# guptakhil/show-tell

Hardware: AMD Instinct MI355X
Metric: training images/sec (ResNet101+GRU, emb=512, bs=128) at 1/2/4/8 MI355X (higher is better)
Workload: dtype bf16; 1 GPU; BASELINE configs[1]: ResNet-101 (train-mode BN, frozen) + 5-layer GRU decoder, E=H=512, V=10000, fwd+bwd+SGD step, synthetic COCO-shaped batch; batch_per_gpu=128, global_batch=128, image=3x224x224, parallelism=dp1

## Files before the change

### show-tell_amd/csrc/rnn.cpp

```cpp
#include "common.h"
#include "rnn_kernels.h"
#include <string.h>
#include <vector>

namespace {

inline size_t al(size_t v) { return (v + 255) & ~(size_t)255; }
inline int up8(int v) { return (v + 7) & ~7; }

struct Plan {
  int G, GH, Np, Vp, maxw;
  size_t es;
  size_t x0, y, gates, cst, dyl, dx0, dgx, dgh, dhc, dcc, tA, tB, wT, wThh, wTih, gA, gB, total;
};

Plan make_plan(const st_rnn_params* p, const st_packed_seq* s) {
  Plan q;
  q.G = p->cell == ST_CELL_GRU ? 3 : 4;
  q.GH = q.G * p->H;
  q.Np = up8(s->ntok);
  q.Vp = st_rnn_vocab_ld(p->V);
  q.es = st_dtype_size(p->dtype);
  q.maxw = p->in0 > p->H ? p->in0 : p->H;
  const size_t n = s->ntok, L = p->L, H = p->H;
  size_t o = 0;
  auto take = [&](size_t bytes) { size_t r = o; o += al(bytes); return r; };
  q.x0 = take(n * p->in0 * q.es);
  q.y = take(L * n * H * q.es);
  q.gates = take(L * n * 4 * H * q.es);
  q.cst = take(p->cell == ST_CELL_LSTM ? L * n * H * q.es : 0);
  q.dyl = take(L * n * H * sizeof(float));
  q.dx0 = take(n * p->in0 * sizeof(float));
  q.dgx = take(L * n * q.GH * q.es);
  q.dgh = take(p->cell == ST_CELL_GRU ? L * n * q.GH * q.es : 0);
  q.dhc = take(L * (size_t)s->B * H * sizeof(float));
  q.dcc = take(L * (size_t)s->B * H * sizeof(float));
  const size_t ra = (size_t)(p->V > q.GH ? p->V : q.GH);
  q.tA = take(ra * q.Np * q.es);
  q.tB = take((size_t)q.maxw * q.Np * q.es);
  const size_t w1 = (size_t)H * q.Vp, w2 = (size_t)q.maxw * q.GH;
  q.wT = take((w1 > w2 ? w1 : w2) * q.es);
  q.wThh = take(L * H * q.GH * q.es);
  q.wTih = take(L * (size_t)q.maxw * q.GH * q.es);
  q.gA = take(2 * L * (size_t)q.GH * q.Np * q.es);
  q.gB = take(2 * L * (size_t)q.maxw * q.Np * q.es);
  q.total = o;
  return q;
}

int gemm_nt(const void* a, int lda, const void* w, int ldw, void* y, int ldy, int M, int N, int K, int dtype, int out_dtype,
            const float* bias, int accumulate, void* stream, int split_k = 0) {
  if (M <= 0 || N <= 0) return 0;
  st_conv_desc d;
  memset(&d, 0, sizeof(d));
  d.split_k = split_k;
  d.x = a; d.w = w; d.y = y; d.bias = bias; d.dtype = dtype; d.out_dtype = out_dtype;
  d.B = M; d.Hin = 1; d.Win = 1; d.Cin = K; d.Ho = 1; d.Wo = 1; d.N = N; d.KH = 1; d.KW = 1; d.stride = 1; d.pad = 0;
  d.ldx = lda; d.ldw = ldw; d.ldy = ldy; d.accumulate = accumulate;
  return st_conv(&d, stream);
}

int check_common(const st_rnn_params* p, const st_packed_seq* s, const char* who) {
  ST_CHECK(p && s, "%s: null descriptor", who);
  ST_CHECK(p->cell == ST_CELL_GRU || p->cell == ST_CELL_LSTM, "%s: bad cell %d", who, p->cell);
  ST_CHECK(p->dtype == ST_F32 || p->dtype == ST_BF16, "%s: bad dtype %d", who, p->dtype);
  ST_CHECK(p->L >= 1 && p->L <= ST_MAX_LAYERS, "%s: num_layers=%d out of range [1,%d]", who, p->L, ST_MAX_LAYERS);
  ST_CHECK(p->H % 8 == 0 && p->in0 % 8 == 0 && p->E % 8 == 0, "%s: E=%d, in0=%d and H=%d must be multiples of 8", who, p->E, p->in0, p->H);
  ST_CHECK(p->V > 0, "%s: bad vocabulary size", who);
  ST_CHECK(s->B > 0 && s->T > 0 && s->ntok > 0 && s->batch_sizes_host && s->rows_b && s->rows_t && s->prev_row && s->caption,
           "%s: bad packed-sequence descriptor", who);
  int sum = 0, prev = s->B;
  for (int t = 0; t < s->T; ++t) {
    const int b = s->batch_sizes_host[t];
    ST_CHECK(b > 0 && b <= prev, "%s: batch_sizes must be positive and non-increasing (captions sorted by length, utils.py:66)", who);
    prev = b; sum += b;
  }
  ST_CHECK(sum == s->ntok && s->batch_sizes_host[0] == s->B, "%s: batch_sizes do not add up to ntok", who);
  for (int l = 0; l < p->L; ++l)
    ST_CHECK(p->w_ih[l] && p->w_hh[l] && p->b_ih[l] && p->b_hh[l], "%s: null weights for layer %d", who, l);
  return 0;
}

}

// ... 75 lines not shown
  ST_CHECK(workspace && targets && scratch && loss_accum, "st_rnn_fused_loss: null pointer");
  ST_CHECK(st_rnn_fused_loss_supported(p), "st_rnn_fused_loss: needs bf16, H = 512 and the vocabulary projection (use st_rnn_forward's logits + st_cross_entropy)");
  const Plan q = make_plan(p, s);
  ST_CHECK(workspace_bytes >= q.total && scratch_bytes >= st_rnn_fused_loss_bytes(p, s), "st_rnn_fused_loss: workspace / scratch too small");
  const char* ytop = reinterpret_cast<const char*>(workspace) + q.y + (size_t)(p->L - 1) * s->ntok * p->H * q.es;
  const int n = s->ntok;
  return vocab_ce_forward(ytop, p->w_lin, p->b_lin, targets, n, p->V, scratch + 2 * (size_t)n, scratch + n, scratch, loss_accum,
                          reinterpret_cast<hipStream_t>(stream));
}
extern "C" int st_rnn_fused_dlogits(const st_rnn_params* p, const st_packed_seq* s, const void* workspace, size_t workspace_bytes,
                                    const long* targets, const float* scratch, const float* grad_scale_dev, void* dlogits, int ldd, void* stream) {
  if (check_common(p, s, "st_rnn_fused_dlogits")) return 1;
  ST_CHECK(workspace && targets && scratch && dlogits, "st_rnn_fused_dlogits: null pointer");
  ST_CHECK(st_rnn_fused_loss_supported(p), "st_rnn_fused_dlogits: unsupported configuration");
  const Plan q = make_plan(p, s);
  ST_CHECK(workspace_bytes >= q.total, "st_rnn_fused_dlogits: workspace too small");
  const char* ytop = reinterpret_cast<const char*>(workspace) + q.y + (size_t)(p->L - 1) * s->ntok * p->H * q.es;
  return vocab_ce_dlogits(ytop, p->w_lin, p->b_lin, targets, scratch, s->ntok, p->V, dlogits, ldd, 1.0f, grad_scale_dev,
                          reinterpret_cast<hipStream_t>(stream));
}

extern "C" int st_rnn_backward(const st_rnn_params* p, const st_rnn_grads* g, const st_packed_seq* s,
                               const void* x0_override, const void* dlogits, int ldd, const float* dy_top_extra,
                               void* workspace, size_t workspace_bytes, float* dfeat, float* dx0_out, void* stream) {
  if (check_common(p, s, "st_rnn_backward")) return 1;
  ST_CHECK(g && workspace, "st_rnn_backward: null pointer");
  const Plan q = make_plan(p, s);
  ST_CHECK(workspace_bytes >= q.total, "st_rnn_backward: workspace too small (%zu < %zu)", workspace_bytes, q.total);
  hipStream_t st = reinterpret_cast<hipStream_t>(stream);
  char* ws = reinterpret_cast<char*>(workspace);
  const int dt = p->dtype, H = p->H, n = s->ntok, Np = q.Np, GH = q.GH;
  const size_t es = q.es;
  std::vector<int> off(s->T + 1, 0);
  for (int t = 0; t < s->T; ++t) off[t + 1] = off[t] + s->batch_sizes_host[t];
  const int L = p->L, T = s->T;
  auto dyl = [&](int l) { return reinterpret_cast<float*>(ws + q.dyl) + (size_t)l * n * H; };
  float* dy = dyl(L - 1);
  const char* ytop = ws + q.y + (size_t)(p->L - 1) * n * H * es;

  if (dlogits) {
    ST_CHECK(p->w_lin && g->w_lin && g->b_lin, "st_rnn_backward: vocabulary projection gradients requested without buffers");
    ST_CHECK(ldd >= up8(p->V) && ldd % 8 == 0 && ldd <= q.Vp, "st_rnn_backward: dlogits leading dimension %d must be a multiple of 8 in [%d, %d]",
             ldd, up8(p->V), q.Vp);
    if (st_transpose_colsum(dlogits, ws + q.tA, g->b_lin, dt, n, p->V, ldd, Np, stream)) return 1;
    if (st_transpose(ytop, ws + q.tB, dt, n, H, H, Np, stream)) return 1;
    if (gemm_nt(ws + q.tA, Np, ws + q.tB, Np, g->w_lin, H, p->V, H, Np, dt, ST_F32, nullptr, 1, stream)) return 1;
    if (st_transpose(p->w_lin, ws + q.wT, dt, p->V, H, H, ldd, stream)) return 1;
    const int bk = dt == ST_BF16 ? 64 : 32;
    const int split = (ldd % (8 * bk) == 0 && ldd >= 16 * bk) ? 8 : 0;
    if (gemm_nt(dlogits, ldd, ws + q.wT, ldd, dy, H, n, H, ldd, dt, ST_F32, nullptr, 0, stream, split)) return 1;
    if (dy_top_extra) { st_set_error("st_rnn_backward: dlogits and dy_top_extra are exclusive"); return 1; }
  } else {
    ST_CHECK(dy_top_extra, "st_rnn_backward: need dlogits or dy_top");
    if (hipMemcpyAsync(dy, dy_top_extra, (size_t)n * H * sizeof(float), hipMemcpyDeviceToDevice, st) != hipSuccess) {
      st_set_error("st_rnn_backward: copy failed"); return 1;
    }
  }

  const void* x0 = x0_override ? x0_override : ws + q.x0;
  const bool need_dx0 = dfeat || dx0_out || g->emb;
  float* dx0 = dx0_out ? dx0_out : reinterpret_cast<float*>(ws + q.dx0);
  const bool gru = p->cell == ST_CELL_GRU;
  auto dgxl = [&](int l) { return ws + q.dgx + (size_t)l * n * GH * es; };
  auto dghl = [&](int l) { return gru ? ws + q.dgh + (size_t)l * n * GH * es : dgxl(l); };
  auto dhcl = [&](int l) { return reinterpret_cast<float*>(ws + q.dhc) + (size_t)l * s->B * H; };
  auto dccl = [&](int l) { return reinterpret_cast<float*>(ws + q.dcc) + (size_t)l * s->B * H; };
  auto wThh = [&](int l) { return ws + q.wThh + (size_t)l * H * GH * es; };
  auto wTih = [&](int l) { return ws + q.wTih + (size_t)l * q.maxw * GH * es; };
  if (hipMemsetAsync(ws + q.dhc, 0, (size_t)L * s->B * H * sizeof(float), st) != hipSuccess ||
      hipMemsetAsync(ws + q.dcc, 0, (size_t)L * s->B * H * sizeof(float), st) != hipSuccess) { st_set_error("memset failed"); return 1; }
  {
    const void* wx[2][ST_MAX_LAYERS]; void* wy[2][ST_MAX_LAYERS];
    int ni = 0;
    for (int l = 0; l < L; ++l) {
      const int in = l == 0 ? p->in0 : H;
      wx[0][l] = p->w_hh[l]; wy[0][l] = wThh(l);
      if (!(l > 0 || need_dx0)) continue;
      if (in == H) { wx[1][ni] = p->w_ih[l]; wy[1][ni] = wTih(l); ++ni; }
      else if (st_transpose(p->w_ih[l], wTih(l), dt, GH, in, in, GH, stream)) return 1;
    }
    if (st_transpose_batch(wx[0], wy[0], nullptr, L, dt, GH, H, H, GH, nullptr, nullptr, stream)) return 1;
    if (ni && st_transpose_batch(wx[1], wy[1], nullptr, ni, dt, GH, H, H, GH, nullptr, nullptr, stream)) return 1;
  }
  for (int d = T + L - 2; d >= 0; --d) {
    RnnBwdCell gc[ST_MAX_LAYERS];
    RnnGemmArgs mc[2 * ST_MAX_LAYERS];
    int ng = 0, nm = 0;
    for (int l = d < T ? 0 : d - (T - 1); l <= d && l < L; ++l) {
      const int t = d - l;
      const int bt = s->batch_sizes_host[t];
      const int in = l == 0 ? p->in0 : H;
      char* yl = ws + q.y + (size_t)l * n * H * es;
      char* gl = ws + q.gates + (size_t)l * n * 4 * H * es;
      char* cl = ws + q.cst + (size_t)l * n * H * es;
      RnnBwdCell& c = gc[ng++];
      memset(&c, 0, sizeof(c));
      c.dy = dyl(l) + (size_t)off[t] * H; c.dhc = dhcl(l); c.dcc = dccl(l);
      c.cache = gl + (size_t)off[t] * 4 * H * es;
      c.hprev = t > 0 ? yl + (size_t)off[t - 1] * H * es : nullptr;
      c.cnew = cl + (size_t)off[t] * H * es;
      c.cprev = t > 0 ? cl + (size_t)off[t - 1] * H * es : nullptr;
      c.dgx = dgxl(l) + (size_t)off[t] * GH * es; c.dgh = dghl(l) + (size_t)off[t] * GH * es; c.Bt = bt;
      if (t > 0) {
        RnnGemmArgs& a = mc[nm++];
        memset(&a, 0, sizeof(a));
        a.A = dghl(l) + (size_t)off[t] * GH * es; a.W = wThh(l); a.M = bt; a.N = H; a.K = GH; a.lda = GH; a.ldw = GH;
        a.out_f32 = dhcl(l); a.ldo = H; a.accumulate = 1;
      }
      if (l > 0 || need_dx0) {
        RnnGemmArgs& a = mc[nm++];
        memset(&a, 0, sizeof(a));
        a.A = dgxl(l) + (size_t)off[t] * GH * es; a.W = wTih(l); a.M = bt; a.N = in; a.K = GH; a.lda = GH; a.ldw = GH;
        a.out_f32 = (l > 0 ? dyl(l - 1) + (size_t)off[t] * H : dx0 + (size_t)off[t] * in); a.ldo = in;
      }
    }
    if (rnn_bwd_gates_launch_batch(gc, ng, H, p->cell, dt, st)) return 1;
    if (rnn_gemm_launch_batch(mc, nm, dt, 0, 0, st)) return 1;
  }
  st_conv_desc gd[2 * ST_MAX_LAYERS];
  int ng = 0;
  auto wgrad = [&](const void* aT, const void* bT, float* dw, int rows, int cols) {
    st_conv_desc& d = gd[ng++];
    memset(&d, 0, sizeof(d));
    d.x = aT; d.w = bT; d.y = dw; d.dtype = dt; d.out_dtype = ST_F32;
    d.B = rows; d.Hin = 1; d.Win = 1; d.Cin = Np; d.Ho = 1; d.Wo = 1; d.N = cols; d.KH = 1; d.KW = 1; d.stride = 1; d.pad = 0;
    d.ldx = Np; d.ldw = Np; d.ldy = cols; d.accumulate = 1;
  };
  const void* tx[4][ST_MAX_LAYERS]; void* ty[4][ST_MAX_LAYERS]; float* tc[4][ST_MAX_LAYERS];
  int nx = 0;
  for (int l = 0; l < L; ++l) {
    const int in = l == 0 ? p->in0 : H;
    const char* xl = l == 0 ? reinterpret_cast<const char*>(x0) : ws + q.y + (size_t)(l - 1) * n * H * es;
    char* aIh = ws + q.gA + (size_t)(2 * l) * GH * Np * es;
    char* aHh = ws + q.gA + (size_t)(2 * l + 1) * GH * Np * es;
    char* bIh = ws + q.gB + (size_t)(2 * l) * q.maxw * Np * es;
    char* bHh = ws + q.gB + (size_t)(2 * l + 1) * q.maxw * Np * es;
    tx[0][l] = dgxl(l); ty[0][l] = aIh; tc[0][l] = g->b_ih[l];
    tx[2][l] = dghl(l); ty[2][l] = aHh; tc[2][l] = g->b_hh[l];
    tx[3][l] = ws + q.y + (size_t)l * n * H * es; ty[3][l] = bHh; tc[3][l] = nullptr;
    if (in == H) {
      tx[1][nx] = xl; ty[1][nx] = bIh; tc[1][nx] = nullptr; ++nx;
      wgrad(aIh, bIh, g->w_ih[l], GH, in);
    } else {
      if (st_transpose(xl, bIh, dt, n, in, in, Np, stream)) return 1;
    }
    wgrad(gru ? aHh : aIh, bHh, g->w_hh[l], GH, H);
    if (!gru && colsum_launch(dghl(l), g->b_hh[l], n, GH, GH, dt, st)) return 1;
  }
  if (st_transpose_batch(tx[0], ty[0], tc[0], L, dt, n, GH, GH, Np, nullptr, nullptr, stream)) return 1;
  if (nx && st_transpose_batch(tx[1], ty[1], nullptr, nx, dt, n, H, H, Np, nullptr, nullptr, stream)) return 1;
  if (gru && st_transpose_batch(tx[2], ty[2], tc[2], L, dt, n, GH, GH, Np, nullptr, nullptr, stream)) return 1;
  if (st_transpose_batch(tx[3], ty[3], nullptr, L, dt, n, H, H, Np, s->rows_t, s->prev_row, stream)) return 1;
  for (int l = 0; l < L; ++l) {
    const int in = l == 0 ? p->in0 : H;
    if (in != H && gemm_nt(ws + q.gA + (size_t)(2 * l) * GH * Np * es, Np, ws + q.gB + (size_t)(2 * l) * q.maxw * Np * es, Np,
                           g->w_ih[l], in, GH, in, Np, dt, ST_F32, nullptr, 1, stream)) return 1;
  }
  for (int i = 0; i < ng; i += 12) {
    if (st_conv_batch(gd + i, ng - i < 12 ? ng - i : 12, stream)) return 1;
  }
  if (need_dx0 && !x0_override) {
    ST_CHECK(g->emb, "st_rnn_backward: embedding gradient buffer missing");
    if (embedding_bwd_launch(dx0, s->caption, s->Tcap, s->rows_b, s->rows_t, dfeat, g->emb, n, p->E, p->V, 0, st)) return 1;
  }
  return 0;
}
```

### show-tell_amd/csrc/rnn_kernels.h

```cpp
#pragma once
#include "common.h"

struct RnnGemmArgs {
  const void* A; const void* W; int M, N, K, lda, ldw, gstride;
  const void* A2; const void* W2; int K2, lda2, ldw2;
  float* out_f32; int ldo; int accumulate;
  const float* bias_h; const float* bias_x;
  const void* gx; int ldgx;
  const void* hprev; const void* cprev; int ldhp;
  void* hout; void* cout; int ldho;
  void* hout2; int ldho2;
  void* cache; int ldcache;
  unsigned long long* argmax_keys;
  const unsigned long long* x_keys; int x_V;
  long* ids_out; int ids_stride, ids_t;
};
constexpr int kCellRawOut = 1, kCellSplit = 2;

constexpr int kRnnBatch = 16;
struct RnnGemmBatch { RnnGemmArgs c[kRnnBatch]; };
static_assert(sizeof(RnnGemmBatch) <= 4000, "kernel-argument segment is 4 KiB");
struct RnnBwdCell {
  const float* dy; float* dhc; float* dcc; const void* cache; const void* hprev; const void* cnew; const void* cprev;
  void* dgx; void* dgh; int Bt;
};
struct RnnBwdBatch { RnnBwdCell c[kRnnBatch]; };

#ifdef __HIPCC__
__device__ __forceinline__ float st_sigm(float x) { return 1.0f / (1.0f + expf(-x)); }
__device__ __forceinline__ float st_gru_unit(float xr, float xz, float xn, float hr, float hz, float hn, float hprev, float& r, float& z, float& n) {
  r = st_sigm(xr + hr);
  z = st_sigm(xz + hz);
  n = tanhf(__builtin_fmaf(r, hn, xn));
  return __builtin_fmaf(z, hprev, (1.f - z) * n);
}
__device__ __forceinline__ float st_lstm_unit(float pi, float pf, float pg, float po, float cprev, float& ig, float& fg, float& gg, float& og, float& cn) {
  ig = st_sigm(pi); fg = st_sigm(pf); gg = tanhf(pg); og = st_sigm(po);
  cn = __builtin_fmaf(fg, cprev, ig * gg);
  return og * tanhf(cn);
}
#endif

size_t rnn_greedy_pipe_bytes(const st_rnn_params* p, int B, int steps);
int rnn_greedy_pipe(const st_rnn_params* p, const void* feat, int B, int steps, void* ws, size_t ws_bytes, long* ids_out, hipStream_t st);

int vocab_ce_supported(int dtype, int H);
int vocab_ce_tiles(int V);
int vocab_ce_forward(const void* y, const void* w, const float* bias, const long* target, int n, int V, float* partial, float* tgt,
                     float* lse, float* loss, hipStream_t st);
int vocab_ce_dlogits(const void* y, const void* w, const float* bias, const long* target, const float* lse, int n, int V,
                     void* dlogits, int ldd, float gscale, const float* gscale_dev, hipStream_t st);

int rnn_gemm_launch(const RnnGemmArgs& a, int dtype, int epi, int has_x, hipStream_t st);
int rnn_gemm_launch_batch(const RnnGemmArgs* cells, int ncells, int dtype, int epi, int has_x, hipStream_t st);
int rnn_bwd_gates_launch_batch(const RnnBwdCell* cells, int ncells, int H, int cell_kind, int dtype, hipStream_t st);
int pack_inputs_launch(const void* feat, const void* emb, const long* cap, int Tcap, const int* rows_b, const int* rows_t,
                       void* x0, long* target, int ntok, int E, int V, int mode, int dtype, hipStream_t st);
int embedding_bwd_launch(const float* dx0, const long* cap, int Tcap, const int* rows_b, const int* rows_t,
                         float* dfeat, float* demb, int ntok, int E, int V, int mode, hipStream_t st);
int gather_hprev_launch(const void* y, const int* rows_t, const int* prev_row, void* hp, int ntok, int H, int dtype, hipStream_t st,
                        const void* h0 = nullptr, const int* rows_b = nullptr);
int gru_bwd_gates_launch(const float* dy, float* dhc, const void* cache, const void* hprev, void* dgx, void* dgh,
                         int Bt, int H, int dtype, hipStream_t st);
int lstm_bwd_gates_launch(const float* dy, float* dhc, float* dcc, const void* cache, const void* cnew, const void* cprev,
                          void* dg, int Bt, int H, int dtype, hipStream_t st);
int colsum_launch(const void* x, float* out, int rows, int cols, int ldx, int dtype, hipStream_t st);
```

### show-tell_amd/csrc/rnn_kernels.hip

```cpp
#include "common.h"
#include "rnn_kernels.h"
#include <string.h>

namespace {

template <typename T> struct Mfma;
template <> struct Mfma<bf16_t> {
  static constexpr int EPC = 8;
  static __device__ __forceinline__ void run(const u32x4& a, const u32x4& b, f32x4& c) {
    c = __builtin_amdgcn_mfma_f32_16x16x32_bf16(*reinterpret_cast<const bf16x8*>(&a),
                                                *reinterpret_cast<const bf16x8*>(&b), c, 0, 0, 0);
  }
};
template <> struct Mfma<float> {
  static constexpr int EPC = 4;
  static __device__ __forceinline__ void run(const u32x4& a, const u32x4& b, f32x4& c) {
#pragma unroll
    for (int e = 0; e < 4; ++e)
      c = __builtin_amdgcn_mfma_f32_16x16x4f32(__uint_as_float(a[e]), __uint_as_float(b[e]), c, 0, 0, 0);
  }
};

template <typename T> __device__ __forceinline__ void load4(const T* p, float* v);
template <> __device__ __forceinline__ void load4<float>(const float* p, float* v) {
  const f32x4 t = *reinterpret_cast<const f32x4*>(p);
  v[0] = t[0]; v[1] = t[1]; v[2] = t[2]; v[3] = t[3];
}
template <> __device__ __forceinline__ void load4<bf16_t>(const bf16_t* p, float* v) {
  const u32x2 t = *reinterpret_cast<const u32x2*>(p);
  v[0] = __uint_as_float(t[0] << 16); v[1] = __uint_as_float(t[0] & 0xffff0000u);
  v[2] = __uint_as_float(t[1] << 16); v[3] = __uint_as_float(t[1] & 0xffff0000u);
}
template <typename T> __device__ __forceinline__ void store4(T* p, const float* v);
template <> __device__ __forceinline__ void store4<float>(float* p, const float* v) {
  *reinterpret_cast<f32x4*>(p) = f32x4{v[0], v[1], v[2], v[3]};
}
template <> __device__ __forceinline__ void store4<bf16_t>(bf16_t* p, const float* v) {
  *reinterpret_cast<u32x2*>(p) = u32x2{pack_bf16x2(v[0], v[1]), pack_bf16x2(v[2], v[3])};
}

__device__ __forceinline__ float sigm(float x) { return 1.0f / (1.0f + expf(-x)); }

template <typename T, int NG, bool HAS_X, int MT>
__device__ __forceinline__ void skinny_mma(const RnnGemmArgs& a, int mbase, int n0, int r16, int q4, int kslice,
                                           f32x4 (&accH)[MT][NG], f32x4 (&accX)[MT][NG]) {
  constexpr int EPC = Mfma<T>::EPC;
  constexpr int UNR = (HAS_X && MT == 2) ? 2 : 4;
  const int n = n0 + r16;
  const bool nok = n < a.N;
  const bool hasH = a.A != nullptr, hasX = HAS_X && a.A2 != nullptr;
  const T* WH = reinterpret_cast<const T*>(a.W) + (long)n * a.ldw;
  const long gsH = (long)a.gstride * a.ldw;
  const T* WX = reinterpret_cast<const T*>(a.W2) + (long)n * a.ldw2;
  const long gsX = (long)a.gstride * a.ldw2;
  const T* AH[MT]; const T* AX[MT]; bool mok[MT];
#pragma unroll
  for (int t = 0; t < MT; ++t) {
    const int m = mbase + t * 16 + r16;
    mok[t] = m < a.M;
    AH[t] = reinterpret_cast<const T*>(a.A) + (long)m * a.lda;
    if (!HAS_X && a.x_keys && a.A) {
      int tok = 0;
      if (mok[t]) {
        tok = (int)(0xffffffffu - (unsigned)(a.x_keys[m] & 0xffffffffull));
        if (tok < 0 || tok >= a.x_V) tok = 0;
        if (a.ids_out && n0 == 0 && kslice == 0 && q4 == 0) a.ids_out[(long)m * a.ids_stride + a.ids_t] = tok;
      }
      AH[t] = reinterpret_cast<const T*>(a.A) + (long)tok * a.lda;
    }
    long xrow = m;
    if (HAS_X && a.x_keys) {
      int tok = 0;
      if (mok[t]) {
        tok = (int)(0xffffffffu - (unsigned)(a.x_keys[m] & 0xffffffffull));
        if (tok < 0 || tok >= a.x_V) tok = 0;
        if (a.ids_out && n0 == 0 && kslice == 0 && q4 == 0) a.ids_out[(long)m * a.ids_stride + a.ids_t] = tok;
      }
      xrow = tok;
    }
    AX[t] = reinterpret_cast<const T*>(a.A2) + xrow * a.lda2;
  }
  const int nsH = hasH ? (a.K + 4 * EPC - 1) / (4 * EPC) : 0, nsX = hasX ? (a.K2 + 4 * EPC - 1) / (4 * EPC) : 0;
  const int spwH = (nsH + 3) / 4, spwX = (nsX + 3) / 4;
  const int begH = kslice * spwH, endH = min(nsH, begH + spwH), begX = kslice * spwX, endX = min(nsX, begX + spwX);
  const int ngroups = max((endH - begH + UNR - 1) / UNR, (endX - begX + UNR - 1) / UNR);
  for (int gi = 0; gi < ngroups; ++gi) {
    u32x4 fa[MT][UNR], fw[UNR][NG], xa[MT][UNR], xw[UNR][NG];
#pragma unroll
    for (int u = 0; u < UNR; ++u) {
      const int sH = begH + gi * UNR + u, kH = (sH * 4 + q4) * EPC;
      const bool okH = sH < endH && kH < a.K;
#pragma unroll
      for (int t = 0; t < MT; ++t) {
        fa[t][u] = u32x4{0u, 0u, 0u, 0u};
        if (mok[t] && okH) fa[t][u] = *reinterpret_cast<const u32x4*>(AH[t] + kH);
      }
#pragma unroll
      for (int g = 0; g < NG; ++g) {
        fw[u][g] = u32x4{0u, 0u, 0u, 0u};
        if (nok && okH) fw[u][g] = *reinterpret_cast<const u32x4*>(WH + g * gsH + kH);
      }
      if (HAS_X) {
        const int sX = begX + gi * UNR + u, kX = (sX * 4 + q4) * EPC;
        const bool okX = sX < endX && kX < a.K2;
#pragma unroll
        for (int t = 0; t < MT; ++t) {
          xa[t][u] = u32x4{0u, 0u, 0u, 0u};
          if (mok[t] && okX) xa[t][u] = *reinterpret_cast<const u32x4*>(AX[t] + kX);
        }
#pragma unroll
        for (int g = 0; g < NG; ++g) {
          xw[u][g] = u32x4{0u, 0u, 0u, 0u};
          if (nok && okX) xw[u][g] = *reinterpret_cast<const u32x4*>(WX + g * gsX + kX);
        }
      }
    }
#pragma unroll
    for (int u = 0; u < UNR; ++u)
#pragma unroll
      for (int g = 0; g < NG; ++g)
#pragma unroll
        for (int t = 0; t < MT; ++t) {
          Mfma<T>::run(fw[u][g], fa[t][u], accH[t][g]);
          if (HAS_X) Mfma<T>::run(xw[u][g], xa[t][u], accX[t][g]);
        }
  }
}

template <typename T, int NG, int EPI, bool HAS_X, int MT>
__global__ __launch_bounds__(256) void rnn_gemm_kernel(RnnGemmBatch batch) {
  const RnnGemmArgs& a = batch.c[blockIdx.z];
  __shared__ f32x4 red[4][MT][2 * NG][64];
  const int lane = threadIdx.x & 63;
  const int wid = __builtin_amdgcn_readfirstlane(threadIdx.x >> 6);
  const int r16 = lane & 15, q4 = lane >> 4;
  const int n0 = blockIdx.x * 16, mbase = blockIdx.y * 16 * MT;
  if (mbase >= a.M || n0 >= a.N) return;
  const int m0 = mbase + (wid < MT ? wid : 0) * 16;
  f32x4 accH[MT][NG], accX[MT][NG];
#pragma unroll
  for (int t = 0; t < MT; ++t)
#pragma unroll
    for (int g = 0; g < NG; ++g) { accH[t][g] = f32x4{0.f, 0.f, 0.f, 0.f}; accX[t][g] = f32x4{0.f, 0.f, 0.f, 0.f}; }
  const int pm = m0 + r16, pn = n0 + 4 * q4;
  const bool epi_ok = wid < MT && pm < a.M && pn < a.N && EPI != 3;
  float ex[NG][4], eb[NG][4], es[4] = {0.f, 0.f, 0.f, 0.f};
#pragma unroll
  for (int g = 0; g < NG; ++g)
#pragma unroll
    for (int e = 0; e < 4; ++e) { ex[g][e] = 0.f; eb[g][e] = 0.f; }
  if (epi_ok) {
    if (EPI == 0) {
      if (a.bias_h) load4<float>(a.bias_h + pn, eb[0]);
      if (a.accumulate) load4<float>(a.out_f32 + (long)pm * a.ldo + pn, es);
    } else {
#pragma unroll
      for (int g = 0; g < NG; ++g) {
        load4<float>(a.bias_h + g * a.N + pn, eb[g]);
        if (HAS_X) load4<float>(a.bias_x + g * a.N + pn, ex[g]);
        else if (a.accumulate == kCellSplit) load4<float>(reinterpret_cast<const float*>(a.gx) + (long)pm * a.ldgx + g * a.N + pn, ex[g]);
        else if (a.accumulate != kCellRawOut) load4<T>(reinterpret_cast<const T*>(a.gx) + (long)pm * a.ldgx + g * a.N + pn, ex[g]);
      }
      const void* prev = EPI == 1 ? a.hprev : a.cprev;
      if (prev && a.accumulate != kCellRawOut) load4<T>(reinterpret_cast<const T*>(prev) + (long)pm * a.ldhp + pn, es);
    }
  }
  skinny_mma<T, NG, HAS_X, MT>(a, mbase, n0, r16, q4, wid, accH, accX);
#pragma unroll
  for (int t = 0; t < MT; ++t)
#pragma unroll
    for (int g = 0; g < NG; ++g) { red[wid][t][g][lane] = accH[t][g]; if (HAS_X) red[wid][t][NG + g][lane] = accX[t][g]; }
  __syncthreads();
  if (wid >= MT) return;
  f32x4 sumH[NG], sumX[NG];
#pragma unroll
  for (int g = 0; g < NG; ++g) {
    sumH[g] = red[0][wid][g][lane];
    if (HAS_X) sumX[g] = red[0][wid][NG + g][lane];
#pragma unroll
    for (int w = 1; w < 4; ++w) {
      sumH[g] += red[w][wid][g][lane];
      if (HAS_X) sumX[g] += red[w][wid][NG + g][lane];
    }
  }

  const int m = m0 + r16, n = n0 + 4 * q4;
  if (EPI != 3 && (m >= a.M || n >= a.N)) return;
  const int H = a.N;
  if (EPI == 3) {
    float best = -INFINITY; int bi = 0x7fffffff;
#pragma unroll
    for (int e = 0; e < 4; ++e) {
      if (n + e < a.N) {
        const float v = sumH[0][e] + (a.bias_h ? a.bias_h[n + e] : 0.f);
        if (v > best) { best = v; bi = n + e; }
      }
    }
// ... 116 lines not shown
    u32x4 v = {0u, 0u, 0u, 0u};
    if (rows_t[row] > 0) v = *reinterpret_cast<const u32x4*>(y + (long)prev_row[row] * H + c);
    else if (h0) v = *reinterpret_cast<const u32x4*>(h0 + (long)rows_b[row] * H + c);
    *reinterpret_cast<u32x4*>(hp + (long)row * H + c) = v;
  }
}

template <typename T>
__global__ __launch_bounds__(256) void gru_bwd_gates_kernel(RnnBwdBatch batch, int H) {
  const RnnBwdCell& cl = batch.c[blockIdx.y];
  const float* __restrict__ dy = cl.dy; float* __restrict__ dhc = cl.dhc;
  const T* __restrict__ cache = reinterpret_cast<const T*>(cl.cache);
  const T* __restrict__ hprev = reinterpret_cast<const T*>(cl.hprev);
  T* __restrict__ dgx = reinterpret_cast<T*>(cl.dgx); T* __restrict__ dgh = reinterpret_cast<T*>(cl.dgh);
  const int Bt = cl.Bt;
  const int total = Bt * (H / 4);
  const int i = blockIdx.x * blockDim.x + threadIdx.x;
  if (i >= total) return;
  const int b = i / (H / 4), j = (i - b * (H / 4)) * 4;
  float g[4], c[4], r[4], z[4], n[4], hn[4], hp[4] = {0.f, 0.f, 0.f, 0.f};
  load4<float>(dy + (long)b * H + j, g);
  load4<float>(dhc + (long)b * H + j, c);
  const T* cr = cache + (long)b * 4 * H + j;
  load4<T>(cr, r); load4<T>(cr + H, z); load4<T>(cr + 2 * H, n); load4<T>(cr + 3 * H, hn);
  if (hprev) load4<T>(hprev + (long)b * H + j, hp);
  float drp[4], dzp[4], dnp[4], dnr[4], dhz[4];
#pragma unroll
  for (int e = 0; e < 4; ++e) {
    const float dh = g[e] + c[e];
    const float dn = dh * (1.f - z[e]);
    const float dz = dh * (hp[e] - n[e]);
    dnp[e] = dn * (1.f - n[e] * n[e]);
    drp[e] = dnp[e] * hn[e] * r[e] * (1.f - r[e]);
    dzp[e] = dz * z[e] * (1.f - z[e]);
    dnr[e] = dnp[e] * r[e];
    dhz[e] = dh * z[e];
  }
  T* ox = dgx + (long)b * 3 * H + j;
  T* oh = dgh + (long)b * 3 * H + j;
  store4<T>(ox, drp); store4<T>(ox + H, dzp); store4<T>(ox + 2 * H, dnp);
  store4<T>(oh, drp); store4<T>(oh + H, dzp); store4<T>(oh + 2 * H, dnr);
  store4<float>(dhc + (long)b * H + j, dhz);
}

template <typename T>
__global__ __launch_bounds__(256) void lstm_bwd_gates_kernel(RnnBwdBatch batch, int H) {
  const RnnBwdCell& cl = batch.c[blockIdx.y];
  const float* __restrict__ dy = cl.dy; float* __restrict__ dhc = cl.dhc; float* __restrict__ dcc = cl.dcc;
  const T* __restrict__ cache = reinterpret_cast<const T*>(cl.cache);
  const T* __restrict__ cnew = reinterpret_cast<const T*>(cl.cnew);
  const T* __restrict__ cprev = reinterpret_cast<const T*>(cl.cprev);
  T* __restrict__ dg = reinterpret_cast<T*>(cl.dgx);
  const int Bt = cl.Bt;
  const int total = Bt * (H / 4);
  const int i = blockIdx.x * blockDim.x + threadIdx.x;
  if (i >= total) return;
  const int b = i / (H / 4), j = (i - b * (H / 4)) * 4;
  float g[4], ch[4], cc[4], ig[4], fg[4], gg[4], og[4], cn[4], cp[4] = {0.f, 0.f, 0.f, 0.f};
  load4<float>(dy + (long)b * H + j, g);
  load4<float>(dhc + (long)b * H + j, ch);
  load4<float>(dcc + (long)b * H + j, cc);
  const T* cr = cache + (long)b * 4 * H + j;
  load4<T>(cr, ig); load4<T>(cr + H, fg); load4<T>(cr + 2 * H, gg); load4<T>(cr + 3 * H, og);
  load4<T>(cnew + (long)b * H + j, cn);
  if (cprev) load4<T>(cprev + (long)b * H + j, cp);
  float di[4], df[4], dgg[4], dob[4], dcp[4], zero[4] = {0.f, 0.f, 0.f, 0.f};
#pragma unroll
  for (int e = 0; e < 4; ++e) {
    const float dh = g[e] + ch[e];
    const float tc = tanhf(cn[e]);
    const float dc = cc[e] + dh * og[e] * (1.f - tc * tc);
    dob[e] = dh * tc * og[e] * (1.f - og[e]);
    di[e] = dc * gg[e] * ig[e] * (1.f - ig[e]);
    df[e] = dc * cp[e] * fg[e] * (1.f - fg[e]);
    dgg[e] = dc * ig[e] * (1.f - gg[e] * gg[e]);
    dcp[e] = dc * fg[e];
  }
  T* o = dg + (long)b * 4 * H + j;
  store4<T>(o, di); store4<T>(o + H, df); store4<T>(o + 2 * H, dgg); store4<T>(o + 3 * H, dob);
  store4<float>(dcc + (long)b * H + j, dcp);
  store4<float>(dhc + (long)b * H + j, zero);
}

template <typename TL, typename TD>
__global__ __launch_bounds__(256) void ce_kernel(const TL* __restrict__ logits, const long* __restrict__ target,
                                                 float* __restrict__ loss, TD* __restrict__ dlogits,
                                                 int V, int ldl, int ldd, float inv_rows, float gscale, const float* __restrict__ gscale_dev) {
  __shared__ float sm[8], ss[8];
  const int row = blockIdx.x;
  const TL* x = logits + (long)row * ldl;
  float m = -INFINITY, s = 0.f;
  for (int i = threadIdx.x; i < V; i += blockDim.x) {
    const float v = to_f32<TL>(x[i]);
    const float nm = fmaxf(m, v);
    s = s * __expf(m - nm) + __expf(v - nm);
    m = nm;
  }
#pragma unroll
  for (int o = 32; o > 0; o >>= 1) {
    const float om = __shfl_xor(m, o, 64), os = __shfl_xor(s, o, 64);
    const float nm = fmaxf(m, om);
    s = (m == -INFINITY ? 0.f : s * __expf(m - nm)) + (om == -INFINITY ? 0.f : os * __expf(om - nm));
    m = nm;
  }
  const int lane = threadIdx.x & 63, wid = threadIdx.x >> 6;
  if (lane == 0) { sm[wid] = m; ss[wid] = s; }
  __syncthreads();
  float M = sm[0], S = ss[0];
  for (int w = 1; w < (int)(blockDim.x >> 6); ++w) {
    const float nm = fmaxf(M, sm[w]);
    S = S * __expf(M - nm) + ss[w] * __expf(sm[w] - nm);
    M = nm;
  }
  long t = target[row];
  t = t < 0 ? 0 : (t >= V ? V - 1 : t);
  const float lse = M + __logf(S);
  const float xt = to_f32<TL>(x[t]);
  __syncthreads();
  if (threadIdx.x == 0 && loss) atomicAdd(loss, (lse - xt) * inv_rows);
  if (dlogits) {
    if (gscale_dev) gscale *= *gscale_dev;
    TD* d = dlogits + (long)row * ldd;
    for (int i = threadIdx.x; i < V; i += blockDim.x) {
      const float p = __expf(to_f32<TL>(x[i]) - lse);
      d[i] = from_f32<TD>((p - (i == t ? 1.f : 0.f)) * gscale);
    }
    for (int i = V + threadIdx.x; i < ldd; i += blockDim.x) d[i] = from_f32<TD>(0.f);
  }
}

template <typename T>
__global__ __launch_bounds__(256) void colsum_kernel(const T* __restrict__ x, float* __restrict__ out, int rows, int cols, int ldx, int rows_per_block) {
  const int n = blockIdx.x * blockDim.x + threadIdx.x;
  if (n >= cols) return;
  const int r0 = blockIdx.y * rows_per_block, r1 = min(rows, r0 + rows_per_block);
  float s = 0.f;
  for (int r = r0; r < r1; ++r) s += to_f32<T>(x[(long)r * ldx + n]);
  atomicAdd(out + n, s);
}

}

int rnn_gemm_launch_batch(const RnnGemmArgs* cells, int ncells, int dtype, int epi, int has_x, hipStream_t st) {
  ST_CHECK(ncells >= 0 && ncells <= kRnnBatch, "rnn_gemm: %d cells in one launch (max %d)", ncells, kRnnBatch);
  RnnGemmBatch b;
  memset(&b, 0, sizeof(b));
  const int epc = dtype == ST_BF16 ? 8 : 4;
  int nc = 0, maxM = 0, maxN = 0;
  for (int i = 0; i < ncells; ++i) {
    const RnnGemmArgs& a = cells[i];
    if (a.M <= 0) continue;
    ST_CHECK(epi == 3 || a.N % 4 == 0, "rnn_gemm: N=%d must be a multiple of 4", a.N);
    ST_CHECK(a.K % epc == 0 && a.lda % epc == 0 && a.ldw % epc == 0, "rnn_gemm: K/lda/ldw must be multiples of %d", epc);
    if (has_x) ST_CHECK(a.K2 % epc == 0 && a.lda2 % epc == 0 && a.ldw2 % epc == 0, "rnn_gemm: K2/lda2/ldw2 must be multiples of %d", epc);
    b.c[nc++] = a;
    if (a.M > maxM) maxM = a.M;
    if (a.N > maxN) maxN = a.N;
  }
  if (nc == 0) return 0;
  const dim3 grid((maxN + 15) / 16, (maxM + 15) / 16, nc), block(256);
  const bool mt2 = (nc >= 2 || maxM >= 512) && maxM > 16 && epi != 3;
  const dim3 grid2((maxN + 15) / 16, (maxM + 31) / 32, nc);
#define RG(T, NG, EPI, HX) do { if (mt2) hipLaunchKernelGGL((rnn_gemm_kernel<T, NG, EPI, HX, 2>), grid2, block, 0, st, b); \
                               else hipLaunchKernelGGL((rnn_gemm_kernel<T, NG, EPI, HX, 1>), grid, block, 0, st, b); } while (0)
  if (dtype == ST_BF16) {
    if (epi == 0) RG(bf16_t, 1, 0, false);
    else if (epi == 3) RG(bf16_t, 1, 3, false);
    else if (epi == 1) { if (has_x) RG(bf16_t, 3, 1, true); else RG(bf16_t, 3, 1, false); }
    else { if (has_x) RG(bf16_t, 4, 2, true); else RG(bf16_t, 4, 2, false); }
  } else {
    if (epi == 0) RG(float, 1, 0, false);
    else if (epi == 3) RG(float, 1, 3, false);
    else if (epi == 1) { if (has_x) RG(float, 3, 1, true); else RG(float, 3, 1, false); }
    else { if (has_x) RG(float, 4, 2, true); else RG(float, 4, 2, false); }
  }
#undef RG
  ST_LAUNCH_CHECK();
  return 0;
}

int rnn_gemm_launch(const RnnGemmArgs& a, int dtype, int epi, int has_x, hipStream_t st) {
  return rnn_gemm_launch_batch(&a, 1, dtype, epi, has_x, st);
}

int rnn_bwd_gates_launch_batch(const RnnBwdCell* cells, int ncells, int H, int cell_kind, int dtype, hipStream_t st) {
  ST_CHECK(ncells >= 0 && ncells <= kRnnBatch, "rnn_bwd_gates: %d cells in one launch (max %d)", ncells, kRnnBatch);
  RnnBwdBatch b;
  memset(&b, 0, sizeof(b));
  int nc = 0, maxB = 0;
  for (int i = 0; i < ncells; ++i) {
    if (cells[i].Bt <= 0) continue;
    b.c[nc++] = cells[i];
    if (cells[i].Bt > maxB) maxB = cells[i].Bt;
  }
  if (nc == 0) return 0;
  const dim3 grid((maxB * (H / 4) + 255) / 256, nc);
  if (cell_kind == ST_CELL_GRU) {
    if (dtype == ST_BF16) hipLaunchKernelGGL(gru_bwd_gates_kernel<bf16_t>, grid, dim3(256), 0, st, b, H);
    else hipLaunchKernelGGL(gru_bwd_gates_kernel<float>, grid, dim3(256), 0, st, b, H);
  } else {
    if (dtype == ST_BF16) hipLaunchKernelGGL(lstm_bwd_gates_kernel<bf16_t>, grid, dim3(256), 0, st, b, H);
    else hipLaunchKernelGGL(lstm_bwd_gates_kernel<float>, grid, dim3(256), 0, st, b, H);
  }
  ST_LAUNCH_CHECK();
  return 0;
}

static inline int grid1d(long work, int threads = 256) {
  long b = (work + threads - 1) / threads;
  return (int)(b < 1 ? 1 : (b > 4096 ? 4096 : b));
}

int pack_inputs_launch(const void* feat, const void* emb, const long* cap, int Tcap, const int* rows_b, const int* rows_t,
                       void* x0, long* target, int ntok, int E, int V, int mode, int dtype, hipStream_t st) {
  if (ntok <= 0) return 0;
  const int n = dtype == ST_BF16 ? 8 : 4;
  ST_CHECK(E % n == 0, "pack_inputs: E=%d must be a multiple of %d", E, n);
  const int grid = grid1d((long)ntok * (E / n));
  if (dtype == ST_BF16) hipLaunchKernelGGL(pack_inputs_kernel<bf16_t>, dim3(grid), dim3(256), 0, st, (const bf16_t*)feat, (const bf16_t*)emb, cap, Tcap, rows_b, rows_t, (bf16_t*)x0, target, ntok, E, V, mode);
  else hipLaunchKernelGGL(pack_inputs_kernel<float>, dim3(grid), dim3(256), 0, st, (const float*)feat, (const float*)emb, cap, Tcap, rows_b, rows_t, (float*)x0, target, ntok, E, V, mode);
  ST_LAUNCH_CHECK();
  return 0;
}

int embedding_bwd_launch(const float* dx0, const long* cap, int Tcap, const int* rows_b, const int* rows_t,
                         float* dfeat, float* demb, int ntok, int E, int V, int mode, hipStream_t st) {
  if (ntok <= 0) return 0;
  hipLaunchKernelGGL(embedding_bwd_kernel, dim3(grid1d((long)ntok * E)), dim3(256), 0, st, dx0, cap, Tcap, rows_b, rows_t, dfeat, demb, ntok, E, V, mode);
  ST_LAUNCH_CHECK();
  return 0;
}

int gather_hprev_launch(const void* y, const int* rows_t, const int* prev_row, void* hp, int ntok, int H, int dtype, hipStream_t st,
                        const void* h0, const int* rows_b) {
  if (ntok <= 0) return 0;
  const int n = dtype == ST_BF16 ? 8 : 4;
  ST_CHECK(H % n == 0, "gather_hprev: H=%d must be a multiple of %d", H, n);
  const int grid = grid1d((long)ntok * (H / n));
  if (dtype == ST_BF16) hipLaunchKernelGGL(gather_hprev_kernel<bf16_t>, dim3(grid), dim3(256), 0, st, (const bf16_t*)y, rows_t, prev_row, (bf16_t*)hp, ntok, H, (const bf16_t*)h0, rows_b);
  else hipLaunchKernelGGL(gather_hprev_kernel<float>, dim3(grid), dim3(256), 0, st, (const float*)y, rows_t, prev_row, (float*)hp, ntok, H, (const float*)h0, rows_b);
  ST_LAUNCH_CHECK();
  return 0;
}

int gru_bwd_gates_launch(const float* dy, float* dhc, const void* cache, const void* hprev, void* dgx, void* dgh,
                         int Bt, int H, int dtype, hipStream_t st) {
  RnnBwdCell c;
  memset(&c, 0, sizeof(c));
  c.dy = dy; c.dhc = dhc; c.cache = cache; c.hprev = hprev; c.dgx = dgx; c.dgh = dgh; c.Bt = Bt;
  return rnn_bwd_gates_launch_batch(&c, 1, H, ST_CELL_GRU, dtype, st);
}

int lstm_bwd_gates_launch(const float* dy, float* dhc, float* dcc, const void* cache, const void* cnew, const void* cprev,
                          void* dg, int Bt, int H, int dtype, hipStream_t st) {
  RnnBwdCell c;
  memset(&c, 0, sizeof(c));
  c.dy = dy; c.dhc = dhc; c.dcc = dcc; c.cache = cache; c.cnew = cnew; c.cprev = cprev; c.dgx = dg; c.Bt = Bt;
  return rnn_bwd_gates_launch_batch(&c, 1, H, ST_CELL_LSTM, dtype, st);
}

int colsum_launch(const void* x, float* out, int rows, int cols, int ldx, int dtype, hipStream_t st) {
  if (rows <= 0 || cols <= 0) return 0;
  const int rpb = 64;
  const dim3 grid((cols + 255) / 256, (rows + rpb - 1) / rpb);
  if (dtype == ST_BF16) hipLaunchKernelGGL(colsum_kernel<bf16_t>, grid, dim3(256), 0, st, (const bf16_t*)x, out, rows, cols, ldx, rpb);
  else hipLaunchKernelGGL(colsum_kernel<float>, grid, dim3(256), 0, st, (const float*)x, out, rows, cols, ldx, rpb);
  ST_LAUNCH_CHECK();
  return 0;
}

extern "C" int st_cross_entropy(const void* logits, int logits_dtype, const long* target, int rows, int V, int ldl,
                                float* loss_accum, void* dlogits, int dlogits_dtype, int ldd, float grad_scale,
                                const float* grad_scale_dev, void* stream) {
  ST_CHECK(logits && target, "st_cross_entropy: null pointer");
  ST_CHECK(rows >= 0 && V > 0 && ldl >= V, "st_cross_entropy: bad shape");
  if (rows == 0) return 0;
  hipStream_t st = reinterpret_cast<hipStream_t>(stream);
  const float inv = 1.0f / rows, gs = grad_scale / rows;
  const dim3 grid(rows), block(256);
  if (logits_dtype == ST_F32 && (dlogits_dtype == ST_F32 || !dlogits))
    hipLaunchKernelGGL((ce_kernel<float, float>), grid, block, 0, st, (const float*)logits, target, loss_accum, (float*)dlogits, V, ldl, ldd, inv, gs, grad_scale_dev);
  else if (logits_dtype == ST_F32)
    hipLaunchKernelGGL((ce_kernel<float, bf16_t>), grid, block, 0, st, (const float*)logits, target, loss_accum, (bf16_t*)dlogits, V, ldl, ldd, inv, gs, grad_scale_dev);
  else if (dlogits_dtype == ST_BF16 || !dlogits)
    hipLaunchKernelGGL((ce_kernel<bf16_t, bf16_t>), grid, block, 0, st, (const bf16_t*)logits, target, loss_accum, (bf16_t*)dlogits, V, ldl, ldd, inv, gs, grad_scale_dev);
// ... 6 lines not shown
```

Before: 31650 images/sec.

## Fuse GRU/LSTM backward recurrent GEMM with gate-gradient epilogue per diagonal

Adds a fused backward kernel that computes, for each wavefront diagonal of (layer, time) cells, the dh contribution from the next timestep's recurrent gradient and the next layer's input gradient via MFMA, then applies the GRU/LSTM gate-gradient math in the same kernel. This replaces the previous sequence of separate batched GEMM and gate kernels per diagonal, cutting launches and the global round-trip of the dh accumulator. The input-layer dx0 gradient is moved to one large GEMM after the loop. The kernel uses a lane-permuted operand layout through ds_bpermute. The old path stays available behind the ST_BPTT_FUSED=0 environment variable.

New measurement: 32290 images/sec (median of 6 runs). 2.0% higher.

```diff
diff --git a/show-tell_amd/csrc/rnn.cpp b/show-tell_amd/csrc/rnn.cpp
--- a/show-tell_amd/csrc/rnn.cpp
+++ b/show-tell_amd/csrc/rnn.cpp
@@ -1,5 +1,6 @@
 #include "common.h"
 #include "rnn_kernels.h"
+#include <stdlib.h>
 #include <string.h>
 #include <vector>
 
@@ -241,7 +242,39 @@
     if (st_transpose_batch(wx[0], wy[0], nullptr, L, dt, GH, H, H, GH, nullptr, nullptr, stream)) return 1;
     if (ni && st_transpose_batch(wx[1], wy[1], nullptr, ni, dt, GH, H, H, GH, nullptr, nullptr, stream)) return 1;
   }
-  for (int d = T + L - 2; d >= 0; --d) {
+  const char* env = getenv("ST_BPTT_FUSED");
+  const bool fused = !(env && env[0] == '0');
+  for (int d = T + L - 2; fused && d >= 0; --d) {
+    RnnBwdFused fc[ST_MAX_LAYERS];
+    int nf = 0;
+    for (int l = d < T ? 0 : d - (T - 1); l <= d && l < L; ++l) {
+      const int t = d - l;
+      const int bt = s->batch_sizes_host[t];
+      char* yl = ws + q.y + (size_t)l * n * H * es;
+      char* gl = ws + q.gates + (size_t)l * n * 4 * H * es;
+      char* cl = ws + q.cst + (size_t)l * n * H * es;
+      RnnBwdFused& f = fc[nf++];
+      memset(&f, 0, sizeof(f));
+      RnnBwdCell& c = f.e;
+      c.dy = l == L - 1 ? dy + (size_t)off[t] * H : nullptr; c.dhc = dhcl(l); c.dcc = dccl(l);
+      c.cache = gl + (size_t)off[t] * 4 * H * es;
+      c.hprev = t > 0 ? yl + (size_t)off[t - 1] * H * es : nullptr;
+      c.cnew = cl + (size_t)off[t] * H * es;
+      c.cprev = t > 0 ? cl + (size_t)off[t - 1] * H * es : nullptr;
+      c.dgx = dgxl(l) + (size_t)off[t] * GH * es; c.dgh = dghl(l) + (size_t)off[t] * GH * es; c.Bt = bt;
+      RnnGemmArgs& a = f.g;
+      a.M = bt; a.N = H;
+      if (t + 1 < T) {
+        a.A = dghl(l) + (size_t)off[t + 1] * GH * es; a.W = wThh(l); a.M2 = s->batch_sizes_host[t + 1]; a.K = GH; a.lda = GH; a.ldw = GH;
+      }
+      if (l + 1 < L) {
+        a.A2 = dgxl(l + 1) + (size_t)off[t] * GH * es; a.W2 = wTih(l + 1); a.K2 = GH; a.lda2 = GH; a.ldw2 = GH;
+      }
+    }
+    if (rnn_bwd_fused_launch_batch(fc, nf, p->cell, dt, st)) return 1;
+  }
+  if (fused && need_dx0 && gemm_nt(dgxl(0), GH, wTih(0), GH, dx0, p->in0, n, p->in0, GH, dt, ST_F32, nullptr, 0, stream)) return 1;
+  for (int d = T + L - 2; !fused && d >= 0; --d) {
     RnnBwdCell gc[ST_MAX_LAYERS];
     RnnGemmArgs mc[2 * ST_MAX_LAYERS];
     int ng = 0, nm = 0;
diff --git a/show-tell_amd/csrc/rnn_kernels.h b/show-tell_amd/csrc/rnn_kernels.h
--- a/show-tell_amd/csrc/rnn_kernels.h
+++ b/show-tell_amd/csrc/rnn_kernels.h
@@ -4,6 +4,7 @@
 struct RnnGemmArgs {
   const void* A; const void* W; int M, N, K, lda, ldw, gstride;
   const void* A2; const void* W2; int K2, lda2, ldw2;
+  int M2;
   float* out_f32; int ldo; int accumulate;
   const float* bias_h; const float* bias_x;
   const void* gx; int ldgx;
@@ -25,6 +26,9 @@
   void* dgx; void* dgh; int Bt;
 };
 struct RnnBwdBatch { RnnBwdCell c[kRnnBatch]; };
+struct RnnBwdFused { RnnGemmArgs g; RnnBwdCell e; };
+struct RnnBwdFusedBatch { RnnBwdFused c[ST_MAX_LAYERS]; };
+static_assert(sizeof(RnnBwdFusedBatch) <= 4000, "kernel-argument segment is 4 KiB");
 
 #ifdef __HIPCC__
 __device__ __forceinline__ float st_sigm(float x) { return 1.0f / (1.0f + expf(-x)); }
@@ -54,6 +58,7 @@
 int rnn_gemm_launch(const RnnGemmArgs& a, int dtype, int epi, int has_x, hipStream_t st);
 int rnn_gemm_launch_batch(const RnnGemmArgs* cells, int ncells, int dtype, int epi, int has_x, hipStream_t st);
 int rnn_bwd_gates_launch_batch(const RnnBwdCell* cells, int ncells, int H, int cell_kind, int dtype, hipStream_t st);
+int rnn_bwd_fused_launch_batch(const RnnBwdFused* cells, int ncells, int cell_kind, int dtype, hipStream_t st);
 int pack_inputs_launch(const void* feat, const void* emb, const long* cap, int Tcap, const int* rows_b, const int* rows_t,
                        void* x0, long* target, int ntok, int E, int V, int mode, int dtype, hipStream_t st);
 int embedding_bwd_launch(const float* dx0, const long* cap, int Tcap, const int* rows_b, const int* rows_t,
diff --git a/show-tell_amd/csrc/rnn_kernels.hip b/show-tell_amd/csrc/rnn_kernels.hip
--- a/show-tell_amd/csrc/rnn_kernels.hip
+++ b/show-tell_amd/csrc/rnn_kernels.hip
@@ -41,23 +41,29 @@
 
 __device__ __forceinline__ float sigm(float x) { return 1.0f / (1.0f + expf(-x)); }
 
-template <typename T, int NG, bool HAS_X, int MT>
+__device__ __forceinline__ u32x4 lane_gather(const u32x4& v, int src4) {
+  return u32x4{(unsigned)__builtin_amdgcn_ds_bpermute(src4, (int)v[0]), (unsigned)__builtin_amdgcn_ds_bpermute(src4, (int)v[1]),
+               (unsigned)__builtin_amdgcn_ds_bpermute(src4, (int)v[2]), (unsigned)__builtin_amdgcn_ds_bpermute(src4, (int)v[3])};
+}
+template <typename T, int NG, bool HAS_X, int MT, bool BWD = false>
 __device__ __forceinline__ void skinny_mma(const RnnGemmArgs& a, int mbase, int n0, int r16, int q4, int kslice,
                                            f32x4 (&accH)[MT][NG], f32x4 (&accX)[MT][NG]) {
   constexpr int EPC = Mfma<T>::EPC;
-  constexpr int UNR = (HAS_X && MT == 2) ? 2 : 4;
-  const int n = n0 + r16;
+  constexpr int UNR = BWD ? (MT + NG <= 4 ? 4 : 2) : (HAS_X && MT == 2) ? 2 : 4;
+  const int lr = BWD ? q4 * 4 + (r16 >> 2) : r16, lq = BWD ? (r16 & 3) : q4;
+  const int n = n0 + lr;
   const bool nok = n < a.N;
   const bool hasH = a.A != nullptr, hasX = HAS_X && a.A2 != nullptr;
   const T* WH = reinterpret_cast<const T*>(a.W) + (long)n * a.ldw;
   const long gsH = (long)a.gstride * a.ldw;
   const T* WX = reinterpret_cast<const T*>(a.W2) + (long)n * a.ldw2;
   const long gsX = (long)a.gstride * a.ldw2;
-  const T* AH[MT]; const T* AX[MT]; bool mok[MT];
+  const T* AH[MT]; const T* AX[MT]; bool mok[MT], mokH[MT];
 #pragma unroll
   for (int t = 0; t < MT; ++t) {
-    const int m = mbase + t * 16 + r16;
+    const int m = mbase + t * 16 + lr;
     mok[t] = m < a.M;
+    mokH[t] = BWD ? m < a.M2 : mok[t];
     AH[t] = reinterpret_cast<const T*>(a.A) + (long)m * a.lda;
     if (!HAS_X && a.x_keys && a.A) {
       int tok = 0;
@@ -88,20 +94,20 @@
     u32x4 fa[MT][UNR], fw[UNR][NG], xa[MT][UNR], xw[UNR][NG];
 #pragma unroll
     for (int u = 0; u < UNR; ++u) {
-      const int sH = begH + gi * UNR + u, kH = (sH * 4 + q4) * EPC;
+      const int sH = begH + gi * UNR + u, kH = (sH * 4 + lq) * EPC;
       const bool okH = sH < endH && kH < a.K;
 #pragma unroll
       for (int t = 0; t < MT; ++t) {
         fa[t][u] = u32x4{0u, 0u, 0u, 0u};
-        if (mok[t] && okH) fa[t][u] = *reinterpret_cast<const u32x4*>(AH[t] + kH);
+        if (mokH[t] && okH) fa[t][u] = *reinterpret_cast<const u32x4*>(AH[t] + kH);
       }
 #pragma unroll
       for (int g = 0; g < NG; ++g) {
         fw[u][g] = u32x4{0u, 0u, 0u, 0u};
-        if (nok && okH) fw[u][g] = *reinterpret_cast<const u32x4*>(WH + g * gsH + kH);
+        if ((BWD ? n + g * 16 < a.N : nok) && okH) fw[u][g] = *reinterpret_cast<const u32x4*>(WH + g * gsH + kH);
       }
       if (HAS_X) {
-        const int sX = begX + gi * UNR + u, kX = (sX * 4 + q4) * EPC;
+        const int sX = begX + gi * UNR + u, kX = (sX * 4 + lq) * EPC;
         const bool okX = sX < endX && kX < a.K2;
 #pragma unroll
         for (int t = 0; t < MT; ++t) {
@@ -111,8 +117,18 @@
 #pragma unroll
         for (int g = 0; g < NG; ++g) {
           xw[u][g] = u32x4{0u, 0u, 0u, 0u};
-          if (nok && okX) xw[u][g] = *reinterpret_cast<const u32x4*>(WX + g * gsX + kX);
+          if ((BWD ? n + g * 16 < a.N : nok) && okX) xw[u][g] = *reinterpret_cast<const u32x4*>(WX + g * gsX + kX);
         }
+      }
+    }
+    if (BWD) {
+      const int src4 = (r16 * 4 + q4) * 4;
+#pragma unroll
+      for (int u = 0; u < UNR; ++u) {
+#pragma unroll
+        for (int t = 0; t < MT; ++t) { fa[t][u] = lane_gather(fa[t][u], src4); xa[t][u] = lane_gather(xa[t][u], src4); }
+#pragma unroll
+        for (int g = 0; g < NG; ++g) { fw[u][g] = lane_gather(fw[u][g], src4); xw[u][g] = lane_gather(xw[u][g], src4); }
       }
     }
 #pragma unroll
@@ -395,6 +411,116 @@
   store4<float>(dhc + (long)b * H + j, zero);
 }
 
+
+template <typename T> struct Raw4;
+template <> struct Raw4<float> { typedef f32x4 type; };
+template <> struct Raw4<bf16_t> { typedef u32x2 type; };
+template <typename T> __device__ __forceinline__ void unpack4(const typename Raw4<T>::type& t, float* v);
+template <> __device__ __forceinline__ void unpack4<float>(const f32x4& t, float* v) { v[0] = t[0]; v[1] = t[1]; v[2] = t[2]; v[3] = t[3]; }
+template <> __device__ __forceinline__ void unpack4<bf16_t>(const u32x2& t, float* v) {
+  v[0] = __uint_as_float(t[0] << 16); v[1] = __uint_as_float(t[0] & 0xffff0000u);
+  v[2] = __uint_as_float(t[1] << 16); v[3] = __uint_as_float(t[1] & 0xffff0000u);
+}
+
+template <typename T, bool LSTM, int MT, int NT>
+__global__ __launch_bounds__(256) void rnn_bwd_cell_kernel(RnnBwdFusedBatch batch) {
+  typedef typename Raw4<T>::type raw_t;
+  const RnnGemmArgs& a = batch.c[blockIdx.z].g;
+  const RnnBwdCell& c = batch.c[blockIdx.z].e;
+  constexpr int TILES = MT * NT, TPW = (TILES + 3) / 4;
+  __shared__ f32x4 red[4][TILES][64];
+  const int lane = threadIdx.x & 63;
+  const int wid = __builtin_amdgcn_readfirstlane(threadIdx.x >> 6);
+  const int r16 = lane & 15, q4 = lane >> 4;
+  const int n0 = blockIdx.x * 16 * NT, mbase = blockIdx.y * 16 * MT;
+  if (mbase >= a.M || n0 >= a.N) return;
+  const int H = a.N;
+  f32x4 accH[MT][NT], accX[MT][NT];
+#pragma unroll
+  for (int t = 0; t < MT; ++t)
+#pragma unroll
+    for (int g = 0; g < NT; ++g) { accH[t][g] = f32x4{0.f, 0.f, 0.f, 0.f}; accX[t][g] = f32x4{0.f, 0.f, 0.f, 0.f}; }
+  bool ok[TPW]; int pm[TPW], pn[TPW];
+  f32x4 rdy[TPW], rdhc[TPW], rdcc[TPW]; raw_t rc[TPW][4], rp[TPW], rcn[TPW];
+  const T* cache = reinterpret_cast<const T*>(c.cache);
+#pragma unroll
+  for (int j = 0; j < TPW; ++j) {
+    const int i = wid + 4 * j;
+    pm[j] = mbase + (i / NT) * 16 + r16; pn[j] = n0 + (i % NT) * 16 + 4 * q4;
+    ok[j] = i < TILES && pm[j] < a.M && pn[j] < H;
+    rdy[j] = rdhc[j] = rdcc[j] = f32x4{0.f, 0.f, 0.f, 0.f};
+    rp[j] = rcn[j] = raw_t{};
+#pragma unroll
+    for (int q = 0; q < 4; ++q) rc[j][q] = raw_t{};
+    if (!ok[j]) continue;
+    const long o = (long)pm[j] * H + pn[j];
+    if (c.dy) rdy[j] = *reinterpret_cast<const f32x4*>(c.dy + o);
+#pragma unroll
+    for (int q = 0; q < 4; ++q) rc[j][q] = *reinterpret_cast<const raw_t*>(cache + (long)pm[j] * 4 * H + q * H + pn[j]);
+    if (LSTM) {
+      rdcc[j] = *reinterpret_cast<const f32x4*>(c.dcc + o);
+      rcn[j] = *reinterpret_cast<const raw_t*>(reinterpret_cast<const T*>(c.cnew) + o);
+      if (c.cprev) rp[j] = *reinterpret_cast<const raw_t*>(reinterpret_cast<const T*>(c.cprev) + o);
+    } else {
+      rdhc[j] = *reinterpret_cast<const f32x4*>(c.dhc + o);
+      if (c.hprev) rp[j] = *reinterpret_cast<const raw_t*>(reinterpret_cast<const T*>(c.hprev) + o);
+    }
+  }
+  skinny_mma<T, NT, true, MT, true>(a, mbase, n0, r16, q4, wid, accH, accX);
+#pragma unroll
+  for (int t = 0; t < MT; ++t)
+#pragma unroll
+    for (int g = 0; g < NT; ++g) red[wid][t * NT + g][lane] = accH[t][g] + accX[t][g];
+  __syncthreads();
+#pragma unroll
+  for (int j = 0; j < TPW; ++j) {
+    if (!ok[j]) continue;
+    const int i = wid + 4 * j;
+    const f32x4 s = ((red[0][i][lane] + red[1][i][lane]) + red[2][i][lane]) + red[3][i][lane];
+    const long o = (long)pm[j] * H + pn[j];
+    if (!LSTM) {
+      float r[4], z[4], n[4], hn[4], hp[4];
+      unpack4<T>(rc[j][0], r); unpack4<T>(rc[j][1], z); unpack4<T>(rc[j][2], n); unpack4<T>(rc[j][3], hn); unpack4<T>(rp[j], hp);
+      float drp[4], dzp[4], dnp[4], dnr[4], dhz[4];
+#pragma unroll
+      for (int e = 0; e < 4; ++e) {
+        const float dh = (rdy[j][e] + rdhc[j][e]) + s[e];
+        const float dn = dh * (1.f - z[e]);
+        const float dz = dh * (hp[e] - n[e]);
+        dnp[e] = dn * (1.f - n[e] * n[e]);
+        drp[e] = dnp[e] * hn[e] * r[e] * (1.f - r[e]);
+        dzp[e] = dz * z[e] * (1.f - z[e]);
+        dnr[e] = dnp[e] * r[e];
+        dhz[e] = dh * z[e];
+      }
+      T* ox = reinterpret_cast<T*>(c.dgx) + (long)pm[j] * 3 * H + pn[j];
+      T* oh = reinterpret_cast<T*>(c.dgh) + (long)pm[j] * 3 * H + pn[j];
+      store4<T>(ox, drp); store4<T>(ox + H, dzp); store4<T>(ox + 2 * H, dnp);
+      store4<T>(oh, drp); store4<T>(oh + H, dzp); store4<T>(oh + 2 * H, dnr);
+      store4<float>(c.dhc + o, dhz);
+    } else {
+      float ig[4], fg[4], gg[4], og[4], cn[4], cp[4];
+      unpack4<T>(rc[j][0], ig); unpack4<T>(rc[j][1], fg); unpack4<T>(rc[j][2], gg); unpack4<T>(rc[j][3], og);
+      unpack4<T>(rcn[j], cn); unpack4<T>(rp[j], cp);
+      float di[4], df[4], dgg[4], dob[4], dcp[4];
+#pragma unroll
+      for (int e = 0; e < 4; ++e) {
+        const float dh = rdy[j][e] + s[e];
+        const float tc = tanhf(cn[e]);
+        const float dc = rdcc[j][e] + dh * og[e] * (1.f - tc * tc);
+        dob[e] = dh * tc * og[e] * (1.f - og[e]);
+        di[e] = dc * gg[e] * ig[e] * (1.f - ig[e]);
+        df[e] = dc * cp[e] * fg[e] * (1.f - fg[e]);
+        dgg[e] = dc * ig[e] * (1.f - gg[e] * gg[e]);
+        dcp[e] = dc * fg[e];
+      }
+      T* og_ = reinterpret_cast<T*>(c.dgx) + (long)pm[j] * 4 * H + pn[j];
+      store4<T>(og_, di); store4<T>(og_ + H, df); store4<T>(og_ + 2 * H, dgg); store4<T>(og_ + 3 * H, dob);
+      store4<float>(c.dcc + o, dcp);
+    }
+  }
+}
+
 template <typename TL, typename TD>
 __global__ __launch_bounds__(256) void ce_kernel(const TL* __restrict__ logits, const long* __restrict__ target,
                                                  float* __restrict__ loss, TD* __restrict__ dlogits,
@@ -514,6 +640,41 @@
   } else {
     if (dtype == ST_BF16) hipLaunchKernelGGL(lstm_bwd_gates_kernel<bf16_t>, grid, dim3(256), 0, st, b, H);
     else hipLaunchKernelGGL(lstm_bwd_gates_kernel<float>, grid, dim3(256), 0, st, b, H);
+  }
+  ST_LAUNCH_CHECK();
+  return 0;
+}
+
+int rnn_bwd_fused_launch_batch(const RnnBwdFused* cells, int ncells, int cell_kind, int dtype, hipStream_t st) {
+  ST_CHECK(ncells >= 0 && ncells <= ST_MAX_LAYERS, "rnn_bwd_fused: %d cells in one launch (max %d)", ncells, ST_MAX_LAYERS);
+  RnnBwdFusedBatch b;
+  memset(&b, 0, sizeof(b));
+  const int epc = dtype == ST_BF16 ? 8 : 4;
+  int nc = 0, maxM = 0, maxN = 0;
+  for (int i = 0; i < ncells; ++i) {
+    const RnnGemmArgs& a = cells[i].g;
+    if (a.M <= 0) continue;
+    ST_CHECK(a.N % 8 == 0, "rnn_bwd_fused: H=%d must be a multiple of 8", a.N);
+    ST_CHECK(!a.A || (a.K % epc == 0 && a.lda % epc == 0 && a.ldw % epc == 0 && a.M2 >= 0 && a.M2 <= a.M),
+             "rnn_bwd_fused: bad recurrent operand pair");
+    ST_CHECK(!a.A2 || (a.K2 % epc == 0 && a.lda2 % epc == 0 && a.ldw2 % epc == 0), "rnn_bwd_fused: bad input operand pair");
+    b.c[nc] = cells[i];
+    b.c[nc].g.gstride = 16;
+    if (!a.A) b.c[nc].g.M2 = 0;
+    ++nc;
+    if (a.M > maxM) maxM = a.M;
+    if (a.N > maxN) maxN = a.N;
+  }
+  if (nc == 0) return 0;
+  const bool lstm = cell_kind == ST_CELL_LSTM;
+  constexpr int MT = 2, NT = 2;
+  const dim3 grid((maxN + 16 * NT - 1) / (16 * NT), (maxM + 16 * MT - 1) / (16 * MT), nc), block(256);
+  if (dtype == ST_BF16) {
+    if (lstm) hipLaunchKernelGGL((rnn_bwd_cell_kernel<bf16_t, true, MT, NT>), grid, block, 0, st, b);
+    else hipLaunchKernelGGL((rnn_bwd_cell_kernel<bf16_t, false, MT, NT>), grid, block, 0, st, b);
+  } else {
+    if (lstm) hipLaunchKernelGGL((rnn_bwd_cell_kernel<float, true, MT, NT>), grid, block, 0, st, b);
+    else hipLaunchKernelGGL((rnn_bwd_cell_kernel<float, false, MT, NT>), grid, block, 0, st, b);
   }
   ST_LAUNCH_CHECK();
   return 0;
```
